# proroklab/VectorizedMultiAgentSimulator

Measured on NVIDIA H100. Metric: env-steps/sec, higher is better.
Workload: dtype f32

## Files before the change

vectorizedmultiagentsimulator_b200/csrc/spec_kernel.cuh:

```cuda
#pragma once
#include <cuda_runtime.h>
#include <stdint.h>

#include <type_traits>
#include <utility>

#include "geometry.cuh"
#include "ingest.cuh"
#include "query.cuh"
#include "vmas_b200.h"

namespace vmas {

struct EntC {
  int shape, flags, agent;
  float d0, d1, mass, inertia, drag_mult, lin_fric, ang_fric, grav_x, grav_y, max_speed, v_range, max_f, f_range,
      max_t, t_range, circ_r, r_plus_lmd;
  float inertia_k0, inertia_k1;
};
struct ItemC {
  int kind, a, b, flags, mask_bit;
  float dmin_base, ax, ay, bx, by, dist, fixed_rot, broad_thr;
};
struct CfgC {
// ... 893 lines not shown
          constexpr int k = decltype(ki)::value;
          constexpr ObsColC col = P::obs[row * F + c0 + k];
          v[k] = 0.f;
          if constexpr (col.op == VMAS_OBS_REG) {
            v[k] = pr[col.src];
          } else if constexpr (col.op != VMAS_OBS_SKIP) {
            v[k] = epi_state<W, (col.src >> 24) & 3, col.src & 0xFFFFFF>(r, a, env);
            if constexpr (col.op == VMAS_OBS_DIFF)
              v[k] = v[k] - epi_state<W, (col.src2 >> 24) & 3, col.src2 & 0xFFFFFF>(r, a, env);
            if constexpr (col.op == VMAS_OBS_REMAINDER) v[k] = obs_remainder(v[k], col.par);
          } else {
            all = false;
          }
          if constexpr (DT != VMAS_DTYPE_F32 && k % 2 == 1) packed[k / 2] = obs16x2_bits<DT>(v[k - 1], v[k]);
        });
        if constexpr (DT == VMAS_DTYPE_F32) {
          if constexpr (VEC == 4) {
            if (all) {
              *reinterpret_cast<float4*>(dst + c0) = make_float4(v[0], v[1], v[2], v[3]);
              return;
            }
          }
        } else if constexpr (VEC == 2) {
          if (all) {
            *reinterpret_cast<uint32_t*>(dst16 + c0) = packed[0];
            return;
          }
        }
        static_for<VEC>([&](auto ki) {
          constexpr int k = decltype(ki)::value;
          if constexpr (P::obs[row * F + c0 + k].op != VMAS_OBS_SKIP) {
            if constexpr (DT == VMAS_DTYPE_F32) dst[c0 + k] = v[k];
            else dst16[c0 + k] = obs16_bits<DT>(v[k]);
          }
        });
      });
    });
  }
}

template <class W, bool TRACK = false, class P = void>
DEVI void spec_env_step(const SpecArgs& a, const long env, const uint32_t (&mask_words)[W::MASK_WORDS > 0 ? W::MASK_WORDS : 1],
                        const EpiArgs* epi = nullptr) {
  constexpr int E = W::E, NA = W::A, NI = W::NI;
  if (env >= a.batch_dim) return;
  SpecRows<W> rows;
  rows.load_pos_rot(a, env);
  rows.load_rest(a, env);
  if constexpr (!std::is_void_v<P>) {
    if (a.first_substep + a.n_substeps == W::cfg.substeps) spec_epilogue_prefetch<P>(*epi, env);
  }
  EnvRegs<E> r;
  float afx[NA > 0 ? NA : 1], afy[NA > 0 ? NA : 1], atq[NA > 0 ? NA : 1];
  rows.unpack_pos_rot(r);
  rows.unpack_rest(r, afx, afy, atq);
  SpecEnvParams<W> pe;
  if constexpr (SpecPerEnv<W>::any) pe.load(a, env);
  uint32_t sig = 0;
  for (int sub = a.first_substep; sub < a.first_substep + a.n_substeps; ++sub) {
    spec_trig<W>(r);
    spec_entity_forces<W>(r, afx, afy, atq, &pe);
    static_for<NI>([&](auto ii) { spec_item<W, decltype(ii)::value, TRACK>(r, a, env, mask_words, sig); });
    spec_integrate<W>(r, sub, &pe);
  }
  rows.store(a, env, r, afx, afy, atq);
  if constexpr (!std::is_void_v<P>) {
    if (a.first_substep + a.n_substeps == W::cfg.substeps) spec_epilogue<W, P>(r, a, *epi, env);
  }
  if constexpr (TRACK) {
    if (a.sig) a.sig[env] = (a.first_substep == 0 ? 0u : a.sig[env]) | sig;
  }
}

template <class P, int G, int J>
struct SpecActRound {
  static constexpr int k0 = J * G, k1 = k0 + G - 1 < P::N_ACT ? k0 + G - 1 : k0;
};

template <class P, int G, int J>
DEVI float2 spec_ingest_lane(const ActArgs& act, const long env, const bool odd, const bool live, bool& bad) {
  constexpr int k0 = SpecActRound<P, G, J>::k0, k1 = SpecActRound<P, G, J>::k1;
  constexpr ActC c0 = P::act[k0], c1 = P::act[k1];
  static_assert(c0.kind == c1.kind, "one action kind per round");
  const bool o = k0 != k1 && odd;
  const float range0 = o ? c1.range0 : c0.range0, range1 = o ? c1.range1 : c0.range1;
  float2 u;
  if constexpr (c0.kind == VMAS_ACT_CONTINUOUS) {
    const float2 v = reinterpret_cast<const float2*>(o ? act.actions[k1] : act.actions[k0])[env];
    const float ux = ingest_continuous(v.x, range0, o ? c1.mult0 : c0.mult0, act.clamp, bad);
    u = make_float2(ux, ingest_continuous(v.y, range1, o ? c1.mult1 : c0.mult1, act.clamp, bad));
  } else {
    const void* in = o ? act.actions[k1] : act.actions[k0];
    const long long n1 = o ? c1.n1 : c0.n1;
    long long i0, i1;
    if constexpr (c0.kind == VMAS_ACT_DISCRETE) {
      const long long flat = static_cast<const long long*>(in)[env];
      i0 = flat / n1;
      i1 = flat % n1;
    } else {
      const ActIdx2 k = static_cast<const ActIdx2*>(in)[env];
      i0 = k.i0;
      i1 = k.i1;
    }
    const float ux = ingest_discrete(i0, o ? c1.n0 : c0.n0, range0, o ? c1.mult0 : c0.mult0, bad);
    u = make_float2(ux, ingest_discrete(i1, n1, range1, o ? c1.mult1 : c0.mult1, bad));
  }
  if (live && (k0 != k1 || !odd)) reinterpret_cast<float2*>(o ? act.u[k1] : act.u[k0])[env] = u;
  return u;
}

template <class P, int G, int J>
DEVI void spec_ingest_put(const float2 u, const float2 p, const bool odd, float* afx, float* afy) {
  constexpr int k0 = SpecActRound<P, G, J>::k0, k1 = SpecActRound<P, G, J>::k1;
  constexpr ActC c0 = P::act[k0], c1 = P::act[k1];
  if constexpr (k0 == k1) {
    afx[c0.agent] = u.x;
    afy[c0.agent] = u.y;
  } else {
    afx[c0.agent] = odd ? p.x : u.x;
    afy[c0.agent] = odd ? p.y : u.y;
    afx[c1.agent] = odd ? u.x : p.x;
    afy[c1.agent] = odd ? u.y : p.y;
  }
}

struct ActBody {
  float rot, w;
  float2 vel;
};
struct ActOut {
  float2 f;
  float t;
};

template <class P>
__host__ __device__ constexpr uint64_t spec_act_cols(bool torque) {
  uint64_t m = 0;
  for (int k = 0; k < P::N_ACT; ++k) {
    const ActC& c = P::act[k];
    if (torque ? dyn_writes_torque(c.dyn) : dyn_writes_force(c.dyn)) m |= (torque ? 1ull : 3ull) << ((torque ? 1 : 2) * c.agent);
  }
  return m;
}
template <class P, int G, int J>
__host__ __device__ constexpr bool spec_act_lean() {
  constexpr ActC c0 = P::act[SpecActRound<P, G, J>::k0], c1 = P::act[SpecActRound<P, G, J>::k1];
  return act_holonomic2(c0) && act_holonomic2(c1) && c0.kind == c1.kind;
}

template <class P, int k, class Body>
DEVI ActOut spec_act_agent(const ActArgs& act, const long env, const bool store_u, bool& bad, Body&& body) {
  constexpr ActC c = P::act[k];
  constexpr int sz = c.size;
  float u[VMAS_MAX_ACTION_SIZE];
  if constexpr (c.kind == VMAS_ACT_CONTINUOUS) {
    const float* in = act.actions[k] + (size_t)env * sz;
    static_for<sz>([&](auto ji) {
      constexpr int j = decltype(ji)::value;
      u[j] = ingest_continuous(in[j], act_range(c, j), act_mult(c, j), act.clamp, bad);
    });
  } else {
    const long long* idx_in = reinterpret_cast<const long long*>(act.actions[k]);
    long long flat = c.kind == VMAS_ACT_DISCRETE ? idx_in[env] : 0;
    static_for<sz>([&](auto ji) {
      constexpr int j = decltype(ji)::value;
      constexpr ActC c = P::act[k];
      long long i;
      if constexpr (c.kind == VMAS_ACT_DISCRETE) {
        long long stride = 1;
        for (int m = j + 1; m < sz; ++m) stride *= act_n(c, m);
        i = flat / stride;
        flat = flat % stride;
      } else {
        i = idx_in[(size_t)env * sz + j];
      }
      u[j] = ingest_discrete(i, act_n(c, j), act_range(c, j), act_mult(c, j), bad);
    });
  }
  ActOut o;
  o.f = make_float2(0.f, 0.f);
  o.t = 0.f;
  if constexpr (c.dyn == VMAS_DYN_HOLONOMIC || c.dyn == VMAS_DYN_HOLONOMIC_ROT) {
    o.f = make_float2(u[0], u[1]);
    if constexpr (c.dyn == VMAS_DYN_HOLONOMIC_ROT) o.t = u[2];
  } else if constexpr (c.dyn == VMAS_DYN_FORWARD) {
    o.f = forward_force(u[0], body(std::integral_constant<int, k>{}).rot);
  } else if constexpr (c.dyn == VMAS_DYN_ROTATION) {
    o.t = u[0];
  } else {
    static_assert(c.dyn == VMAS_DYN_DIFF_DRIVE, "an action model the prologue has not (codegen.PROLOGUE_MODELS)");
    const ActBody b = body(std::integral_constant<int, k>{});
    const float dt = c.params[0], mass = c.params[1], inertia = c.params[2];
    constexpr bool rk4 = c.params[3] != 0.f;
    const Pose3 d = diff_drive_pose(u[0], u[1], b.rot, dt, rk4);
    o.f = kinematic_force(d, dt, mass, inertia, b.vel, b.w, o.t);
  }
  if (store_u) {
    static_for<sz>([&](auto ji) {
      constexpr int j = decltype(ji)::value;
      act.u[k][(size_t)env * sz + j] = u[j];
    });
  }
  return o;
}

template <class P, int G, int J, class Body>
DEVI ActOut spec_act_lane(const ActArgs& act, const long env, const bool odd, const bool live, bool& bad, Body&& body) {
  constexpr int k0 = SpecActRound<P, G, J>::k0, k1 = SpecActRound<P, G, J>::k1;
  if constexpr (k0 == k1) {
    return spec_act_agent<P, k0>(act, env, live && !odd, bad, body);
  } else {
    if (odd) return spec_act_agent<P, k1>(act, env, live, bad, body);
    return spec_act_agent<P, k0>(act, env, live, bad, body);
  }
}

template <class P, int G, int J>
DEVI void spec_act_put(const ActOut& own, const ActOut& p, const bool odd, float* afx, float* afy, float* atq) {
  constexpr int k0 = SpecActRound<P, G, J>::k0, k1 = SpecActRound<P, G, J>::k1;
  constexpr ActC c0 = P::act[k0], c1 = P::act[k1];
  const ActOut& r0 = k0 == k1 || !odd ? own : p;
  if constexpr (dyn_writes_force(c0.dyn)) {
    afx[c0.agent] = r0.f.x;
    afy[c0.agent] = r0.f.y;
  }
  if constexpr (dyn_writes_torque(c0.dyn)) atq[c0.agent] = r0.t;
  if constexpr (k0 != k1) {
    const ActOut& r1 = odd ? own : p;
    if constexpr (dyn_writes_force(c1.dyn)) {
      afx[c1.agent] = r1.f.x;
      afy[c1.agent] = r1.f.y;
    }
    if constexpr (dyn_writes_torque(c1.dyn)) atq[c1.agent] = r1.t;
  }
}

#ifdef __CUDACC__
template <class W, bool SCHED = false>
__global__ void __launch_bounds__(W::BLOCK, W::MIN_BLOCKS) step_spec_kernel(const SpecArgs a) {
  constexpr int MW = W::MASK_WORDS;
  const long tid = (long)blockIdx.x * W::BLOCK + threadIdx.x;

  uint32_t mask_words[MW > 0 ? MW : 1];
  if constexpr (MW > 0) {
    __shared__ uint32_t s_mask[MW];
    if (a.use_mask) {
      for (int w = threadIdx.x; w < MW; w += W::BLOCK) s_mask[w] = a.mask[w];
      __syncthreads();
      if (threadIdx.x == 0) {
        __threadfence();
        unsigned done = atomicAdd(&a.mask[MW], 1u);
        if (done == gridDim.x - 1) {
          for (int w = 0; w < MW; ++w) a.mask[w] = 0u;
          a.mask[MW] = 0u;
        }
      }
#pragma unroll
      for (int w = 0; w < MW; ++w) mask_words[w] = s_mask[w];
    }
  }
  if (tid >= a.batch_dim) return;
  if constexpr (SCHED) {
    const long env = a.order ? (long)a.order[tid] : tid;
    spec_env_step<W, true>(a, env, mask_words);
  } else {
    spec_env_step<W, false>(a, tid, mask_words);
  }
}

template <class W, class P>
__global__ void __launch_bounds__(W::BLOCK, W::MIN_BLOCKS) step_fused_kernel(const SpecArgs a, const EpiArgs e) {
  static_assert(!SpecPerEnv<W>::any, "no whole-step kernel for worlds with per-env parameters");
  constexpr int MW = W::MASK_WORDS;
  const long tid = (long)blockIdx.x * W::BLOCK + threadIdx.x;
  uint32_t mask_words[MW > 0 ? MW : 1];
  if constexpr (MW > 0) {
    __shared__ uint32_t s_mask[MW];
    if (a.use_mask) {
      for (int w = threadIdx.x; w < MW; w += W::BLOCK) s_mask[w] = a.mask[w];
      __syncthreads();
      if (threadIdx.x == 0) {
        __threadfence();
        unsigned done = atomicAdd(&a.mask[MW], 1u);
        if (done == gridDim.x - 1) {
          for (int w = 0; w < MW; ++w) a.mask[w] = 0u;
          a.mask[MW] = 0u;
        }
      }
#pragma unroll
      for (int w = 0; w < MW; ++w) mask_words[w] = s_mask[w];
    }
  }
  if (tid >= a.batch_dim) return;
  spec_env_step<W, false, P>(a, tid, mask_words, &e);
}

template <class W>
__host__ __device__ constexpr int spec_first_masked() {
  for (int i = 0; i < W::NI; ++i)
    if (W::item[i].mask_bit >= 0) return i;
  return W::NI;
}

DEVI unsigned ld_acquire_u32(const uint32_t* p) {
  unsigned v;
  asm volatile("ld.acquire.gpu.global.u32 %0, [%1];" : "=r"(v) : "l"(p) : "memory");
  return v;
}

template <class W>
__host__ __device__ constexpr int spec_masked_item(int k) {
  for (int i = 0; i < W::NI; ++i)
    if (W::item[i].mask_bit >= 0 && k-- == 0) return i;
  return -1;
}
template <class W>
__host__ __device__ constexpr int spec_n_masked() {
  int n = 0;
  for (int i = 0; i < W::NI; ++i) n += W::item[i].mask_bit >= 0;
  return n;
}

template <class W>
__host__ __device__ constexpr int spec_agent_entity(int agent) {
  for (int e = 0; e < W::E; ++e)
    if ((W::ent[e].flags & VMAS_F_AGENT) && W::ent[e].agent == agent) return e;
  return -1;
}

DEVI float pair_swap(float v) { return __shfl_xor_sync(0xffffffffu, v, 1); }

template <class W, int G, int K>
DEVI ItemOut spec_round_swap(const ItemOut& o) {
  constexpr int I0 = SpecRounds<W, G>::template I0<K>, I1 = SpecRounds<W, G>::template I1<K>;
  if constexpr (I0 == I1) {
    return o;
  } else {
    constexpr int fa = W::ent[W::item[I0].a].flags | W::ent[W::item[I1].a].flags;
    constexpr int fb = W::ent[W::item[I0].b].flags | W::ent[W::item[I1].b].flags;
    ItemOut p = o;
    if constexpr ((fa | fb) & VMAS_F_MOVABLE) {
      p.f.x = pair_swap(o.f.x);
      p.f.y = pair_swap(o.f.y);
    }
    if constexpr (fa & VMAS_F_ROTATABLE) p.ta = pair_swap(o.ta);
    if constexpr (fb & VMAS_F_ROTATABLE) p.tb = pair_swap(o.tb);
    return p;
  }
}

template <class W, class P, int G>
__global__ void __launch_bounds__(W::BLOCK* G, (W::MIN_BLOCKS / G > 0 ? W::MIN_BLOCKS / G : 1))
    step_env_kernel(const SpecArgs a, const EpiArgs e, const ActArgs act) {
  static_assert(!SpecPerEnv<W>::any, "no whole-step kernel for worlds with per-env parameters");
  constexpr int MW = W::MASK_WORDS, E = W::E, NA = W::A;
  using R = SpecRounds<W, G>;
  const long tid = ((long)blockIdx.x * (W::BLOCK * G) + threadIdx.x) / G;
  const bool odd = G > 1 && (threadIdx.x & 1);
  const bool live = tid < a.batch_dim;
  const long env = live ? tid : (long)a.batch_dim - 1;
  SpecRows<W, true, spec_act_cols<P>(false), spec_act_cols<P>(true)> rows;
  rows.load_pos_rot(a, env);
  rows.load_rest(a, env);
  spec_epilogue_prefetch<P>(e, env);
#ifdef __CUDA_ARCH__
  if (act.steps) spec_prefetch(act.steps + env);
#endif
  EnvRegs<E> r;
  float afx[NA > 0 ? NA : 1], afy[NA > 0 ? NA : 1], atq[NA > 0 ? NA : 1];
  rows.unpack_pos_rot(r);
  rows.unpack_rest(r, afx, afy, atq);
  bool bad = false;
  static_for<(P::N_ACT + G - 1) / G>([&](auto ji) {
    constexpr int J = decltype(ji)::value;
    constexpr int k0 = SpecActRound<P, G, J>::k0, k1 = SpecActRound<P, G, J>::k1;
    if constexpr (spec_act_lean<P, G, J>()) {
      const float2 u = spec_ingest_lane<P, G, J>(act, env, odd, live, bad);
      if constexpr (k0 == k1)
        spec_ingest_put<P, G, J>(u, u, odd, afx, afy);
      else
        spec_ingest_put<P, G, J>(u, make_float2(pair_swap(u.x), pair_swap(u.y)), odd, afx, afy);
    } else {
      auto body = [&](auto ki) {
        constexpr int ent = spec_agent_entity<W>(P::act[decltype(ki)::value].agent);
        constexpr int f = W::ent[ent].flags;
        const size_t at = (size_t)env * E + ent;
        ActBody b;
        if constexpr (f & (VMAS_F_TRIG | VMAS_F_ROTATABLE)) b.rot = r.rot[ent];
        else b.rot = a.st.rot[at];
        if constexpr (f & VMAS_F_ROTATABLE) b.w = r.w[ent];
        else b.w = a.st.ang_vel[at];
        if constexpr (f & VMAS_F_MOVABLE) b.vel = make_float2(r.vx[ent], r.vy[ent]);
        else b.vel = reinterpret_cast<const float2*>(a.st.vel)[at];
        return b;
      };
      const ActOut own = spec_act_lane<P, G, J>(act, env, odd, live, bad, body);
      ActOut p = own;
      if constexpr (k0 != k1) {
        constexpr ActC c0 = P::act[k0], c1 = P::act[k1];
        if constexpr (dyn_writes_force(c0.dyn) || dyn_writes_force(c1.dyn)) p.f = make_float2(pair_swap(own.f.x), pair_swap(own.f.y));
        if constexpr (dyn_writes_torque(c0.dyn) || dyn_writes_torque(c1.dyn)) p.t = pair_swap(own.t);
      }
      spec_act_put<P, G, J>(own, p, odd, afx, afy, atq);
    }
  });
  if constexpr (G > 1) bad = __shfl_xor_sync(0xffffffffu, (int)bad, 1) || bad;
  if (live && !odd) {
    if (bad && act.bad_flag) *act.bad_flag = 1;
    if (act.steps) act.steps[env] = act.steps[env] + 1.f;
  }
  uint32_t mask_words[MW > 0 ? MW : 1];
  [[maybe_unused]] __shared__ uint32_t s_mask[MW > 0 ? MW : 1];
  static_assert(MW <= W::BLOCK, "more mask words than threads in a block");
  uint32_t sig = 0;
  for (int sub = 0; sub < W::cfg.substeps; ++sub) {
    [[maybe_unused]] uint32_t* gmask = a.mask + sub * (MW + 2);
    if constexpr (MW > 0) {
      if (a.use_mask) {
        if (sub > 0) __syncthreads();
        if (threadIdx.x < MW) s_mask[threadIdx.x] = 0u;
        __syncthreads();
        uint32_t bits[MW];
#pragma unroll
        for (int w = 0; w < MW; ++w) bits[w] = 0u;
        static_for<(spec_n_masked<W>() + G - 1) / G>([&](auto ji) {
          constexpr int j0 = decltype(ji)::value * G, j1 = j0 + G - 1 < spec_n_masked<W>() ? j0 + G - 1 : j0;
          constexpr ItemC i0 = W::item[spec_masked_item<W>(j0)], i1 = W::item[spec_masked_item<W>(j1)];
          const bool o = j0 != j1 && odd;
          const bool near = live && norm2((o ? r.px[i1.a] : r.px[i0.a]) - (o ? r.px[i1.b] : r.px[i0.b]),
                                          (o ? r.py[i1.a] : r.py[i0.a]) - (o ? r.py[i1.b] : r.py[i0.b])) <=
                                        (o ? i1.broad_thr : i0.broad_thr);
          if constexpr (j0 == j1) {
            if (__any_sync(0xffffffffu, near)) bits[i0.mask_bit >> 5] |= 1u << (i0.mask_bit & 31);
          } else {
            const unsigned vote = __ballot_sync(0xffffffffu, near);
            if (vote & 0x55555555u) bits[i0.mask_bit >> 5] |= 1u << (i0.mask_bit & 31);
            if (vote & 0xAAAAAAAAu) bits[i1.mask_bit >> 5] |= 1u << (i1.mask_bit & 31);
          }
        });
        if ((threadIdx.x & 31) == 0) {
#pragma unroll
          for (int w = 0; w < MW; ++w)
            if (bits[w]) atomicOr(&s_mask[w], bits[w]);
        }
        __syncthreads();
        if (threadIdx.x == 0) {
          for (int w = 0; w < MW; ++w) {
            const uint32_t b = s_mask[w];
            if (b && (ld_acquire_u32(&gmask[w]) & b) != b) atomicOr(&gmask[w], b);
          }
          __threadfence();
          atomicAdd(&gmask[MW], 1u);
        }
      }
    }
    static_for<(spec_n_trig<W>() + G - 1) / G>([&](auto ki) {
      constexpr int K = decltype(ki)::value;
      float s, c;
      spec_trig_round_eval<W, G, K>(r, odd, s, c);
      if constexpr (G * K + 1 < spec_n_trig<W>() && G > 1)
        spec_trig_round_put<W, G, K>(r, odd, s, c, pair_swap(s), pair_swap(c));
      else
        spec_trig_round_put<W, G, K>(r, odd, s, c, s, c);
    });
    spec_entity_forces<W>(r, afx, afy, atq);
    static_for<R::N>([&](auto ki) {
      constexpr int K = decltype(ki)::value;
      if constexpr (MW > 0 && R::template I0<K> == spec_first_masked<W>()) {
        if (a.use_mask) {
          if (threadIdx.x == 0) {
            while (ld_acquire_u32(&gmask[MW]) < gridDim.x) __nanosleep(20);
            for (int w = 0; w < MW; ++w) s_mask[w] = ld_acquire_u32(&gmask[w]);
            __threadfence();
            const unsigned done = atomicAdd(&gmask[MW + 1], 1u);
            if (done == gridDim.x - 1) {
              for (int w = 0; w < MW + 2; ++w) gmask[w] = 0u;
            }
          }
          __syncthreads();
#pragma unroll
          for (int w = 0; w < MW; ++w) mask_words[w] = s_mask[w];
        }
      }
      if constexpr (R::template I0<K> == R::template I1<K>) {
        spec_item<W, R::template I0<K>, false>(r, a, env, mask_words, sig);
      } else {
        const ItemOut own = spec_round_eval<W, G, K>(r, a, env, mask_words, odd);
        spec_round_add<W, G, K>(r, a, mask_words, own, spec_round_swap<W, G, K>(own), odd);
      }
    });
    spec_integrate<W>(r, sub);
  }
  if (!live) return;
  rows.store(a, env, r, afx, afy, atq, G, odd ? 1 : 0);
  spec_epilogue<W, P>(r, a, e, env, G, odd ? 1 : 0, [odd](float v) {
    if constexpr (G == 1) return v;
    const float v0 = __shfl_xor_sync(0x3u << (threadIdx.x & 30), v, 1);
    return odd ? v0 : v;
  });
}

template <class W, class P, int G>
static cudaError_t env_capacity(long& cap) {
  static long capacity[64] = {0};
  int device = 0;
  cudaError_t err = cudaGetDevice(&device);
  if (err != cudaSuccess) return err;
  cap = device < 64 ? capacity[device] : 0;
  if (cap == 0) {
    int per_sm = 0, sms = 0;
    err = cudaOccupancyMaxActiveBlocksPerMultiprocessor(&per_sm, step_env_kernel<W, P, G>, W::BLOCK * G, 0);
    if (err != cudaSuccess) return err;
    err = cudaDeviceGetAttribute(&sms, cudaDevAttrMultiProcessorCount, device);
    if (err != cudaSuccess) return err;
    cap = (long)per_sm * sms;
    if (device < 64) capacity[device] = cap;
  }
  return cudaSuccess;
}

template <class W, class P, int G>
static cudaError_t launch_env_lanes(const SpecArgs& a, const EpiArgs& e, const ActArgs& act, long blocks, bool coop,
                                    cudaStream_t stream) {
  if (coop) {
    void* args[] = {const_cast<SpecArgs*>(&a), const_cast<EpiArgs*>(&e), const_cast<ActArgs*>(&act)};
    return cudaLaunchCooperativeKernel(reinterpret_cast<void*>(step_env_kernel<W, P, G>), dim3((unsigned)blocks),
                                       dim3(W::BLOCK * G), args, 0, stream);
  }
  step_env_kernel<W, P, G><<<(unsigned)blocks, W::BLOCK * G, 0, stream>>>(a, e, act);
  return cudaGetLastError();
}

template <class W, class P>
static cudaError_t launch_env(const SpecArgs& a, const EpiArgs& e, const ActArgs& act, cudaStream_t stream) {
  for (int k = 0; k < P::N_ACT; ++k)
    if (act.kind[k] != P::act[k].kind || act.dyn[k] != P::act[k].dyn || act.size[k] != P::act[k].size)
      return cudaErrorInvalidValue;
  const long blocks = ((long)a.batch_dim + W::BLOCK - 1) / W::BLOCK;
  const bool coop = W::MASK_WORDS > 0 && a.use_mask;
  long cap = 0;
  cudaError_t err = env_capacity<W, P, 2>(cap);
  if (err != cudaSuccess) return err;
  if (blocks <= cap) return launch_env_lanes<W, P, 2>(a, e, act, blocks, coop, stream);
  if (coop) {
    err = env_capacity<W, P, 1>(cap);
    if (err != cudaSuccess) return err;
    if (blocks > cap) return cudaErrorCooperativeLaunchTooLarge;
  }
  return launch_env_lanes<W, P, 1>(a, e, act, blocks, coop, stream);
}

template <class W, class P>
static cudaError_t launch_fused(const SpecArgs& a, const EpiArgs& e, cudaStream_t stream) {
  const long blocks = ((long)a.batch_dim + W::BLOCK - 1) / W::BLOCK;
  step_fused_kernel<W, P><<<(unsigned)blocks, W::BLOCK, 0, stream>>>(a, e);
  return cudaGetLastError();
}

template <class W>
static cudaError_t launch_spec(const SpecArgs& a, cudaStream_t stream) {
  if constexpr (spec_needs_params<W>()) {
    if (!a.ent_params) return cudaErrorInvalidValue;
  }
  if constexpr (spec_needs_gravity<W>()) {
    if (!a.ent_gravity) return cudaErrorInvalidValue;
  }
  const long blocks = ((long)a.batch_dim + W::BLOCK - 1) / W::BLOCK;
  if (a.order || a.sig)
    step_spec_kernel<W, true><<<(unsigned)blocks, W::BLOCK, 0, stream>>>(a);
  else
    step_spec_kernel<W, false><<<(unsigned)blocks, W::BLOCK, 0, stream>>>(a);
  return cudaGetLastError();
}
#endif

#ifdef __CUDACC__
struct SpecEntry {
  uint64_t hash;
  const char* name;
  int n_entities, n_items;
  cudaError_t (*launch)(const SpecArgs&, cudaStream_t);
  cudaError_t (*launch_tile)(const SpecArgs&, cudaStream_t);
  bool has_tile;
};
#endif

}
```

Measured before the change: 1.100 billion.

## Skip grid-wide mask barrier when block mask is already full

Each block now checks whether its own broad-phase mask already has every masked item bit set. If so, it uses the local mask and skips the spin-wait on the grid-wide arrival counter. Publishing bits now uses relaxed `red.or` plus a release `red.add` in place of atomics with `__threadfence`. The per-substep reset of the global mask words moves to a single end-of-kernel last-block counter. The aim is to remove grid-wide barrier latency and fence cost from every substep. The risk is that if thread 0 of a block exits early on a non-live env, it never increments the end counter, so the mask would never be reset.

```diff
diff --git a/vectorizedmultiagentsimulator_b200/csrc/spec_kernel.cuh b/vectorizedmultiagentsimulator_b200/csrc/spec_kernel.cuh
--- a/vectorizedmultiagentsimulator_b200/csrc/spec_kernel.cuh
+++ b/vectorizedmultiagentsimulator_b200/csrc/spec_kernel.cuh
@@ -1219,10 +1219,30 @@
   return W::NI;
 }
 
+template <class W>
+__host__ __device__ constexpr uint32_t spec_mask_full(int w) {
+  uint32_t m = 0u;
+  for (int i = 0; i < W::NI; ++i)
+    if (W::item[i].mask_bit >= 0 && (W::item[i].mask_bit >> 5) == w) m |= 1u << (W::item[i].mask_bit & 31);
+  return m;
+}
+
 DEVI unsigned ld_acquire_u32(const uint32_t* p) {
   unsigned v;
   asm volatile("ld.acquire.gpu.global.u32 %0, [%1];" : "=r"(v) : "l"(p) : "memory");
   return v;
+}
+
+DEVI void red_or_u32(uint32_t* p, uint32_t v) {
+  asm volatile("red.relaxed.gpu.global.or.b32 [%0], %1;" ::"l"(p), "r"(v) : "memory");
+}
+DEVI void red_release_add_u32(uint32_t* p, uint32_t v) {
+  asm volatile("red.release.gpu.global.add.u32 [%0], %1;" ::"l"(p), "r"(v) : "memory");
+}
+DEVI unsigned atom_acq_rel_add_u32(uint32_t* p, uint32_t v) {
+  unsigned old;
+  asm volatile("atom.acq_rel.gpu.global.add.u32 %0, [%1], %2;" : "=r"(old) : "l"(p), "r"(v) : "memory");
+  return old;
 }
 
 template <class W>
@@ -1328,6 +1348,7 @@
   }
   uint32_t mask_words[MW > 0 ? MW : 1];
   [[maybe_unused]] __shared__ uint32_t s_mask[MW > 0 ? MW : 1];
+  [[maybe_unused]] __shared__ uint32_t s_gmask[MW > 0 ? MW : 1];
   static_assert(MW <= W::BLOCK, "more mask words than threads in a block");
   uint32_t sig = 0;
   for (int sub = 0; sub < W::cfg.substeps; ++sub) {
@@ -1364,10 +1385,9 @@
         if (threadIdx.x == 0) {
           for (int w = 0; w < MW; ++w) {
             const uint32_t b = s_mask[w];
-            if (b && (ld_acquire_u32(&gmask[w]) & b) != b) atomicOr(&gmask[w], b);
+            if (b) red_or_u32(&gmask[w], b);
           }
-          __threadfence();
-          atomicAdd(&gmask[MW], 1u);
+          red_release_add_u32(&gmask[MW], 1u);
         }
       }
     }
@@ -1385,18 +1405,23 @@
       constexpr int K = decltype(ki)::value;
       if constexpr (MW > 0 && R::template I0<K> == spec_first_masked<W>()) {
         if (a.use_mask) {
-          if (threadIdx.x == 0) {
-            while (ld_acquire_u32(&gmask[MW]) < gridDim.x) __nanosleep(20);
-            for (int w = 0; w < MW; ++w) s_mask[w] = ld_acquire_u32(&gmask[w]);
-            __threadfence();
-            const unsigned done = atomicAdd(&gmask[MW + 1], 1u);
-            if (done == gridDim.x - 1) {
-              for (int w = 0; w < MW + 2; ++w) gmask[w] = 0u;
+          bool full = true;
+          static_for<MW>([&](auto wi) {
+            constexpr uint32_t all = spec_mask_full<W>(decltype(wi)::value);
+            full = full && s_mask[decltype(wi)::value] == all;
+          });
+          if (full) {
+#pragma unroll
+            for (int w = 0; w < MW; ++w) mask_words[w] = s_mask[w];
+          } else {
+            if (threadIdx.x == 0) {
+              while (ld_acquire_u32(&gmask[MW]) < gridDim.x) __nanosleep(20);
+              for (int w = 0; w < MW; ++w) s_gmask[w] = s_mask[w] | ld_acquire_u32(&gmask[w]);
             }
+            __syncthreads();
+#pragma unroll
+            for (int w = 0; w < MW; ++w) mask_words[w] = s_gmask[w];
           }
-          __syncthreads();
-#pragma unroll
-          for (int w = 0; w < MW; ++w) mask_words[w] = s_mask[w];
         }
       }
       if constexpr (R::template I0<K> == R::template I1<K>) {
@@ -1415,6 +1440,13 @@
     const float v0 = __shfl_xor_sync(0x3u << (threadIdx.x & 30), v, 1);
     return odd ? v0 : v;
   });
+  if constexpr (MW > 0) {
+    if (a.use_mask && threadIdx.x == 0) {
+      if (atom_acq_rel_add_u32(&a.mask[MW + 1], 1u) == gridDim.x - 1) {
+        for (int w = 0; w < W::cfg.substeps * (MW + 2); ++w) a.mask[w] = 0u;
+      }
+    }
+  }
 }
 
 template <class W, class P, int G>
```

Measured after the change: 1.191 billion (median of 6 runs). 1.08x the previous value.
